# big-nacho/patolette

Measured on AMD Instinct MI355X. Metric: Mpixels/sec quantized (256-color ICtCp + KMeans) at 1 GPU; palette ΔE vs ref, higher is better.
Workload: dtype f64

## Files before the change

include/patolette_amd.h:

```cpp
#ifndef PATOLETTE_AMD_H
#define PATOLETTE_AMD_H

#include <stddef.h>
#include <stdint.h>

#include "patolette.h"

#ifdef __cplusplus
extern "C" {
#endif

int  patolette_amd_device_count(void);
int  patolette_amd_set_device(int ordinal);
const char *patolette_amd_last_error(void);
void *patolette_amd_malloc(size_t bytes);
void patolette_amd_free(void *dptr);
int  patolette_amd_memcpy_h2d(void *dst, const void *src, size_t bytes);
int  patolette_amd_memcpy_d2h(void *dst, const void *src, size_t bytes);
int  patolette_amd_synchronize(void);
void patolette_amd_release_workspace(void);
int  patolette_amd_fill_image(double *d_planar, size_t n, uint64_t seed);
int  patolette_amd_fill_weights(double *d_weights, size_t n, uint64_t seed);

void patolette_amd_device(size_t width, size_t height, const double *d_data, const double *d_weights,
// ... 182 lines not shown
int patolette_amd_set_invariant_sums(int on);
int patolette_amd_set_kmeans_update(int mode);

int patolette_amd_set_split_loop(int mode);
int patolette_amd_set_global_quantiser(int on_device);

int patolette_amd_set_subsample_cache(int on);

int patolette_amd_subsample_indices(size_t n, size_t take, int32_t *out);
int patolette_amd_eigen_sym3(const double a_colmajor[9], double w[3], double z[9]);
int patolette_amd_principal_axis(const double cov6[6], double axis[3]);
int patolette_amd_eigen_sym3_device(const double *a_colmajor, size_t count, double *w, double *z, int *info);
int patolette_amd_debug_gq_table(const double *table, const uint32_t *counts, int weighted, size_t palette_size, int route, int *kbase, int *error,
                                 int *cuts, unsigned char *bucket_table, uint64_t *begin, uint64_t *n, double *sw, double *mean,
                                 uint64_t *prefix_w0, double *prefix, int *cut_table);
int patolette_amd_pow(const double *x, double y, double *out, size_t n);
int patolette_amd_debug_pow(const double *x, double y, double *out, size_t n, int mode);

enum {
    PAMD_SRGB_TO_ICTCP = 0,
    PAMD_SRGB_TO_CIELUV = 1,
    PAMD_ICTCP_TO_REC2020 = 2,
    PAMD_CIELUV_TO_REC2020 = 3,
    PAMD_SRGB_TO_REC2020 = 4,
    PAMD_REC2020_TO_SRGB = 5,
    PAMD_CIELUV_TO_ICTCP = 6
};
int patolette_amd_convert(int which, double *planar, size_t n);
int patolette_amd_debug_convert(int which, const double *planar, const unsigned char *bytes, int channels, double *out, size_t n, int general);

// ... 76 lines not shown
```

patolette_amd/_native.py:

```python
import ctypes as C
import os

HERE = os.path.dirname(os.path.abspath(__file__))
LIB_PATH = os.path.join(HERE, "lib", "libpatolette_amd.so")

dp = C.POINTER(C.c_double)
zp = C.POINTER(C.c_size_t)


class QuantizationOptions(C.Structure):
    _fields_ = [("dither", C.c_bool), ("palette_only", C.c_bool), ("color_space", C.c_int),
                ("kmeans_niter", C.c_int), ("kmeans_max_samples", C.c_size_t), ("verbose", C.c_bool)]


class Stats(C.Structure):
    _fields_ = [(n, C.c_double) for n in ("ms_total", "ms_upload", "ms_convert", "ms_gq", "ms_lq",
                                          "ms_kmeans", "ms_map", "ms_download", "ms_saliency")] + \
               [(n, C.c_size_t) for n in ("n_base_clusters", "n_clusters", "split_evals", "split_px",
                                          "lq_rounds", "kmeans_samples", "dither_segments", "dither_repairs",
                                          "dither_rounds", "dither_through", "dither_jumps", "dither_solo")]

    def as_dict(self):
        return {n: getattr(self, n) for n, _ in self._fields_}

# ... 40 lines not shown
                                        C.c_size_t, C.POINTER(QuantizationOptions), C.POINTER(dp), C.c_void_p, C.c_int,
                                        C.POINTER(C.c_int)]),
    "patolette_amd_slice": (None, [C.c_size_t, C.c_size_t, C.c_size_t, dp, dp, C.c_size_t, C.POINTER(QuantizationOptions),
                                   C.POINTER(Comm), dp, zp, C.POINTER(C.c_int)]),
    "patolette_amd_slice_device": (None, [C.c_size_t, C.c_size_t, C.c_size_t, C.c_void_p, C.c_void_p, C.c_size_t,
                                          C.POINTER(QuantizationOptions), C.POINTER(Comm), dp, C.c_void_p, C.c_int, C.POINTER(C.c_int)]),
    "patolette_amd_set_invariant_sums": (C.c_int, [C.c_int]),
    "patolette_amd_set_kmeans_update": (C.c_int, [C.c_int]),
    "patolette_amd_set_subsample_cache": (C.c_int, [C.c_int]),
    "patolette_amd_subsample_indices": (C.c_int, [C.c_size_t, C.c_size_t, C.POINTER(C.c_int32)]),
    "patolette_amd_eigen_sym3": (C.c_int, [dp, dp, dp]),
    "patolette_amd_principal_axis": (C.c_int, [dp, dp]),
    "patolette_amd_eigen_sym3_device": (C.c_int, [dp, C.c_size_t, dp, dp, C.POINTER(C.c_int)]),
    "patolette_amd_debug_gq_table": (C.c_int, [dp, C.c_void_p, C.c_int, C.c_size_t, C.c_int, C.POINTER(C.c_int), C.POINTER(C.c_int), C.c_void_p,
                                               C.c_void_p, C.c_void_p, C.c_void_p, dp, dp, C.c_void_p, dp, C.c_void_p]),
    "patolette_amd_fill_image": (C.c_int, [C.c_void_p, C.c_size_t, C.c_uint64]),
    "patolette_amd_fill_weights": (C.c_int, [C.c_void_p, C.c_size_t, C.c_uint64]),
    "patolette_amd_device": (None, [C.c_size_t, C.c_size_t, C.c_void_p, C.c_void_p, C.c_size_t,
                                    C.POINTER(QuantizationOptions), dp, C.c_void_p, C.c_int, C.POINTER(C.c_int)]),
    "patolette_amd_quantize": (None, [C.c_size_t, C.c_size_t, dp, dp, C.c_double, C.c_size_t, C.POINTER(QuantizationOptions), dp, zp,
                                      C.POINTER(C.c_int)]),
    "patolette_amd_quantize_rows": (None, [C.c_size_t, C.c_size_t, dp, dp, C.c_double, C.c_size_t, C.POINTER(QuantizationOptions), dp,
                                           zp, C.POINTER(C.c_int)]),
    "patolette_amd_saliency_weights": (C.c_int, [C.c_size_t, C.c_size_t, dp, C.c_double, dp]),
    "patolette_amd_mbd": (C.c_int, [C.c_size_t, C.c_size_t, C.POINTER(C.c_float), C.c_int, C.POINTER(C.c_float)]),
    **_pair("patolette_amd_u8", None, [C.c_size_t, C.c_size_t, C.c_void_p, C.c_int, C.c_void_p, C.c_double, C.c_size_t,
                                       C.POINTER(QuantizationOptions), dp, C.c_void_p, C.c_void_p, C.c_int, C.c_void_p, C.POINTER(C.c_int)]),
    **_pair("patolette_amd_frames_u8", None, [C.c_size_t, C.c_size_t, C.c_size_t, C.c_void_p, C.c_int, C.c_void_p, C.c_double, C.c_size_t,
                                              C.POINTER(QuantizationOptions), dp, C.c_void_p, C.c_void_p, C.c_int, C.c_void_p,
                                              C.POINTER(C.c_int)]),
# ... 141 lines not shown
    ctab = np.zeros((13, 513), dtype=np.int32) if details else None
    vp = lambda a: a.ctypes.data_as(C.c_void_p) if a is not None else None
    rc = lib().patolette_amd_debug_gq_table(t.ctypes.data_as(dp), vp(c), 1 if weighted else 0, int(palette_size), int(route), C.byref(kbase),
                                            C.byref(error), vp(cuts), vp(lut), vp(begin), vp(n), sw.ctypes.data_as(dp), mean.ctypes.data_as(dp),
                                            vp(pw0), pre.ctypes.data_as(dp) if details else None, vp(ctab))
    if rc != 0:
        raise RuntimeError("patolette_amd_debug_gq_table: %d (%s)" % (rc, last_error()))
    k = kbase.value
    out = dict(kbase=k, error=error.value, cuts=[int(v) for v in cuts[:k + 1]] if k else [], bucket_table=lut, begin=begin[:k].copy(),
               n=n[:k].copy(), sw=sw[:k].copy(), mean=mean[:k].copy())
    if details:
        out.update(prefix_w0=pw0, prefix=pre, cut_table=ctab)
    return out


def last_cluster_centers():
    import numpy as np
    n = lib().patolette_amd_last_cluster_centers(None, 0)
    out = np.zeros((max(1, n), 3), order="F")
    lib().patolette_amd_last_cluster_centers(out.ctypes.data_as(dp), max(1, n))
    return np.ascontiguousarray(out[:n])


def profile(enable=True, only=None, sample=1):
    lib().patolette_amd_profile_only(only.encode() if only else None)
    lib().patolette_amd_profile_sample(int(sample) if only else 1)
    lib().patolette_amd_profile_enable(1 if enable else 0)


def profile_results():
# ... 11 lines not shown
```

patolette_amd/csrc/map.h:

```cpp
#pragma once

#include "common.h"

namespace pamd {

struct NNWork {
    DevBuf<unsigned char> lut;
    DevBuf<unsigned long long> keys;
    DevBuf<unsigned char> clist;
    DevBuf<unsigned int> mid;
    DevBuf<double> dtab;
    DevBuf<unsigned int> dside;
    PinBuf<unsigned int> hrep;
    DevBuf<double> dsort;
    DevBuf<unsigned int> dpos;
    size_t order_w = 0, order_h = 0; int order_dev = -1;
    DevBuf<unsigned int> dmpos;
    DevBuf<unsigned int> dmcnt;
    DevBuf<unsigned char> dsmap;
    DevBuf<unsigned char> dflag;
    size_t dither_segments = 0, dither_repairs = 0, dither_rounds = 0;
    size_t dither_through = 0;
    size_t dither_jumps = 0;
    size_t dither_solo = 0;
// ... 2 lines not shown
    int side_dev = -1;
    struct LaneTables { bool valid = false; double lo[3][3], hi[3][3], inv[3][3]; int G[3]; float amb, amb_p, amb_x; } lane_tables;
    NNWork() = default;
    NNWork(const NNWork &) = delete;
    NNWork &operator=(const NNWork &) = delete;
    ~NNWork() {
        if (ev_fork) (void)hipEventDestroy(ev_fork);
        if (ev_join) (void)hipEventDestroy(ev_join);
        if (ev_join2) (void)hipEventDestroy(ev_join2);
        if (side_stream) (void)hipStreamDestroy(side_stream);
        if (side_stream2) (void)hipStreamDestroy(side_stream2);
    }
};
void launch_nn_map(const double *d_colors, size_t plane_stride, size_t n, const double *d_pal, int k,
                   void *d_out, int elem_bytes, const double *lo, const double *hi, NNWork &w, hipStream_t s);
int nn_debug_route(int route);
bool nn_map_u8_applies(size_t n, int k);
void launch_nn_map_u8(const unsigned char *d_px, int channels, size_t n, const double *d_pal, int k, void *d_out, int elem_bytes, NNWork &w, hipStream_t s);

struct DitherJob {
    const double *planes = nullptr;
    size_t plane_stride = 0;
    int which = -1;
    const unsigned char *bytes = nullptr;
    int channels = 3;
    size_t frames = 1, width = 0, height = 0;
    const int *cpos = nullptr;
    size_t opaque = 0;
    const unsigned *mpos = nullptr;
    const double *d_pal = nullptr, *h_pal = nullptr;
// ... 20 lines not shown
```

patolette_amd/csrc/map.hip:

```cpp
#include "map.h"
#include "compact.h"
#include "dither_host.h"
#include "dither_slots.h"

#include <algorithm>
#include <atomic>
#include <cmath>
#include <mutex>
#include <type_traits>

#define PAMD_POW_TABLES_IN_LDS
#include "color_device.h"
#include "devutil.h"

namespace pamd {

template <typename OutT>
__global__ __launch_bounds__(256) void k_nn_map(const double *__restrict__ c, size_t N, size_t n, const double *__restrict__ pal, int k,
                                                OutT *__restrict__ out) {
    const double *palx = pal, *paly = pal + k, *palz = pal + 2 * k;
    const size_t stride = (size_t)gridDim.x * blockDim.x;
    for (size_t i = (size_t)blockIdx.x * blockDim.x + threadIdx.x; i < n; i += stride) {
        const double x = c[i], y = c[N + i], z = c[2 * N + i];
        double bd = INFINITY; int best = 0;
// ... 788 lines not shown
    const int blocks = (int)std::min<size_t>((size_t)num_cus(), ceil_div(n, (size_t)64 * WAVES * P));
    KTIME("k_nn_map_u8", s, ((double)channels + sizeof(OutT)) * n);
    hipLaunchKernelGGL((k_nn_map_mid<OutT, P, WAVES, NNSrcU8>), blocks, 64 * WAVES, lds, s, NNSrcU8{d_px, (size_t)channels}, n, d_pal, k, g, (const unsigned int *)w.mid.p,
                       (const float4 *)(w.mid.p + ncell / 8), (const unsigned char *)l1, (const unsigned char *)l2, out);
}
void launch_nn_map_u8(const unsigned char *d_px, int channels, size_t n, const double *d_pal, int k, void *d_out, int elem_bytes, NNWork &w, hipStream_t s) {
    if (!nn_map_u8_applies(n, k)) throw HipError("patolette_amd: the byte-source map kernel takes 2^22 .. 2^32 pixels and 8 .. 256 palette rows");
    if (channels != 3 && channels != 4) throw HipError("patolette_amd: 8-bit pixels have 3 or 4 channels");
    w.lane_tables.valid = false;
    if (elem_bytes == 1) launch_nn_mid_u8<unsigned char>(d_px, channels, n, d_pal, k, (unsigned char *)d_out, w, s);
    else if (elem_bytes == 4) launch_nn_mid_u8<unsigned int>(d_px, channels, n, d_pal, k, (unsigned int *)d_out, w, s);
    else throw HipError("patolette_amd: the byte-source map kernel writes 1- or 4-byte elements");
    HIP_CHECK(hipGetLastError());
}

void launch_nn_map(const double *d_colors, size_t plane_stride, size_t n, const double *d_pal, int k, void *d_out, int elem_bytes,
                   const double *lo, const double *hi, NNWork &w, hipStream_t s) {
    if (elem_bytes != 1 && elem_bytes != 4 && elem_bytes != 8) throw HipError("patolette_amd: map element size must be 1, 4 or 8");
    w.lane_tables.valid = false;
    const int cls = nn_size_class(n);
    bool use_lut = cls >= 1 && k >= 8 && k <= 4096;
    double blo[3] = {0, 0, 0}, bhi[3] = {0, 0, 0};
    if (use_lut) {
        if (lo && hi) { for (int a = 0; a < 3; a++) { blo[a] = lo[a]; bhi[a] = hi[a]; } }
        else {
            w.keys.reserve(6);
            unsigned long long init[6] = {~0ULL, ~0ULL, ~0ULL, 0ULL, 0ULL, 0ULL}, got[6];
            HIP_CHECK(hipMemcpyAsync(w.keys.p, init, sizeof init, hipMemcpyHostToDevice, s));
            { KTIME("k_minmax3", s, 24.0 * n); hipLaunchKernelGGL(k_minmax3, stream_blocks(n, 16), 256, 0, s, d_colors, plane_stride, n, w.keys.p); }
            HIP_CHECK(hipMemcpyAsync(got, w.keys.p, sizeof got, hipMemcpyDeviceToHost, s));
// ... 1649 lines not shown
```

patolette_amd/csrc/pipeline.hip:

```cpp
#include <algorithm>
#include <functional>
#include <chrono>
#include <cmath>
#include <atomic>
#include <memory>
#include <mutex>
#include <thread>
#include <future>
#include <type_traits>

#include "color_device.h"
#include "common.h"
#include "host_math.h"
#include "kmeans.h"
#include "map.h"
#include "ordered.h"
#include "delta.h"
#include "measure.h"
#include "lzw.h"
#include "lzw_near.h"
#include "deflate.h"
#include "hist.h"
#include "saliency.h"
#include "quant.h"
// ... 817 lines not shown
    size_t total = 0, begin = 0;
    patolette_amd__Comm comm{};
};

struct Engine {
    int device = -1;
    hipStream_t stream = nullptr;
    const Shard *shard = nullptr;
    bool invariant = false;
    DevBuf<unsigned char> commbuf;
    PinBuf<unsigned char> h_comm;
    DevBuf<int> shard_ids;
    PinBuf<float> h_cent;
    PinBuf<ConvertStats> h_cstats;
    hipEvent_t ev_stats = nullptr;
    hipStream_t stream2 = nullptr;
    hipEvent_t ev_up[2] = {nullptr, nullptr}, ev_join = nullptr;
    size_t prep_N = 0, prep_planes = 0;
    DevBuf<double> src, wsrc, cvt, bufA, bufB, aux;
    DevBuf<unsigned short> bkt;
    DevBuf<NodeDev> nodes;
    DevBuf<NodeIn> stage_in;
    DevBuf<NodeOut> stage_out;
    DevBuf<int> ids, round_nodes, node_tile0;
    DevBuf<Tile> tilesA, tilesP;
    DevBuf<double> hist, sum6, dpal;
    DevBuf<unsigned long long> hsize, tileoff;
    DevBuf<unsigned int> hcount, tilecnt;
    DevBuf<unsigned char> lut, dmap, src8, pal8, quant8;
    DevBuf<unsigned char> dl_maps, dl_shown;
// ... 39 lines not shown
    PinBuf<double> h_pal;
    DevBuf<LqCtl> lqctl;
    PinBuf<LqHead> h_lqhead;
    PinBuf<LqRec> h_lqrec;
    PinBuf<LqCen> h_lqcen;
    std::vector<LqRec> lq_rec_local;
    std::vector<LqCommit> lq_commits;
    bool trace_pending = false;
    size_t lq_hint_N = 0, lq_hint_K = 0; int lq_hint_rounds = 0;
    DevBuf<int> perm_dev;
    size_t perm_N = 0, perm_nx = 0;
    PinBuf<int32_t> h_perm;
    size_t hperm_N = 0, hperm_nx = 0;
    hm::PermScratch perm_ws;
    std::future<void> perm_job;
    patolette_amd__Stats stats{};
    double ms_saliency = 0.0;
    std::string last_error;
    std::vector<double> map_palette;
    patolette_amd__SplitTrace trace_hdr{};
    std::vector<patolette_amd__SplitRecord> trace;
    std::vector<double> cluster_centers;

    void init() {
        if (stream) return;
        int cnt = 0;
        if (hipGetDeviceCount(&cnt) != hipSuccess || cnt <= 0)
            throw HipError("patolette_amd: no HIP device available (this library has no CPU fallback)");
        if (device < 0) { HIP_CHECK(hipGetDevice(&device)); }
        HIP_CHECK(hipSetDevice(device));
        HIP_CHECK(hipStreamCreateWithFlags(&stream, hipStreamNonBlocking));
    }
    void sync() { HIP_CHECK(hipStreamSynchronize(stream)); if (ktimer().enabled) ktimer().collect(); }
    ~Engine() {
        if (stream) { (void)hipSetDevice(device); (void)hipStreamSynchronize(stream); if (ev_stats) (void)hipEventDestroy(ev_stats);
                      for (hipEvent_t e : {ev_up[0], ev_up[1], ev_join}) if (e) (void)hipEventDestroy(e);
                      if (stream2) (void)hipStreamDestroy(stream2);
                      (void)hipStreamDestroy(stream); }
    }
};

namespace {
std::mutex g_pool_mu;
std::vector<Engine *> g_pool;
thread_local int tl_invariant = -1;
bool invariant_default() {
    static const bool env = getenv("PAMD_INVARIANT_SUMS") && atoi(getenv("PAMD_INVARIANT_SUMS")) != 0;
    return tl_invariant < 0 ? env : tl_invariant != 0;
}
Engine *pool_acquire(int device, bool invariant) {
// ... 143 lines not shown

static void get_nodes(Engine &E, const std::vector<int> &ids, std::vector<NodeOut> &recs) {
    const int n = (int)ids.size();
    recs.resize(n);
    if (!n) return;
    E.stage_out.reserve(n); E.ids.reserve(n); E.h_stage_out.reserve(n); E.h_ids_get.reserve(n);
    std::memcpy(E.h_ids_get.p, ids.data(), n * sizeof(int));
    HIP_CHECK(hipMemcpyAsync(E.ids.p, E.h_ids_get.p, n * sizeof(int), hipMemcpyHostToDevice, E.stream));
    hipLaunchKernelGGL(k_get_nodes, (n + 63) / 64, 64, 0, E.stream, E.nodes.p, E.stage_out.p, E.ids.p, n);
    HIP_CHECK(hipGetLastError());
    HIP_CHECK(hipMemcpyAsync(E.h_stage_out.p, E.stage_out.p, n * sizeof(NodeOut), hipMemcpyDeviceToHost, E.stream));
    E.sync();
    std::memcpy(recs.data(), E.h_stage_out.p, n * sizeof(NodeOut));
}

static void get_nodes_dev(Engine &E, const int *d_ids, int n, std::vector<NodeOut> &recs) {
    recs.resize(n);
    if (!n) return;
    E.h_stage_out.reserve(n);
    hipLaunchKernelGGL(k_get_nodes, (n + 63) / 64, 64, 0, E.stream, E.nodes.p, E.h_stage_out.p, d_ids, n);
    HIP_CHECK(hipGetLastError());
    E.sync();
    std::memcpy(recs.data(), E.h_stage_out.p, n * sizeof(NodeOut));
}

static void absorb_moments(HNode &h, const NodeOut &d) {
    for (int q = 0; q < 6; q++) h.cov6[q] = d.acc[q][0] + d.acc[q][1];
    h.dist = d.acc[6][0] + d.acc[6][1];
}

static bool node_axis(const HNode &h, double axis[3]) {
    if (h.axis_state != 0) {
        for (int j = 0; j < 3; j++) axis[j] = h.axis[j];
        return h.axis_state > 0;
    }
    double c6[6];
    for (int q = 0; q < 6; q++) c6[q] = h.cov6[q] / h.sw;
// ... 120 lines not shown
        }
        launch_hist(qlq, false, E.tilesA.p, ntA_ub, 0, E.nodes.p, E.hist.p, E.hsize.p, E.hcount.p, s, !rev, false, dyn, px_src);
        launch_cut(weighted, E.nodes.p, d_round, kLqRoundCap, E.hist.p, E.hsize.p, E.hcount.p, E.lut.p, s, dyn, nr_src);
        launch_partition(qlq, E.tilesP.p, ntP_ub, 0, d_round, d_tP0, kLqRoundCap, E.nodes.p, E.lut.p, E.tilecnt.p, E.tileoff.p, true, s, inv_sums, rev, dyn, px_src);
        enq++;
        control();
    };
    control();
    int want = (E.lq_hint_N == N && E.lq_hint_K == K && E.lq_hint_rounds > 0) ? E.lq_hint_rounds : 9;
    const bool fault_full = g_debug_fault.load(std::memory_order_relaxed) == 4;
    if (fault_full) want = 3;
    for (;;) {
        while (enq < want) round();
        hipLaunchKernelGGL(k_lq_export, 16, 256, 0, s, (const LqCtl *)c, head, E.h_lqrec.p, E.h_lqcen.p);
        HIP_CHECK(hipGetLastError());
        E.sync();
        if (fault_full) return -2;
        if (head->done) break;
        want = enq + 2;
    }
    if (head->error == 2) return -2;
    if (head->error == 3) return -1;
    if (kbase < 0) kbase = E.h_gqout.p->kbase;
    E.lq_hint_N = N; E.lq_hint_K = K; E.lq_hint_rounds = head->rounds;
    LqReplay rp;
    const double t_rp0 = now_ms();
    E.lq_rec_local.resize((size_t)head->nnodes);
    std::memcpy(E.lq_rec_local.data(), E.h_lqrec.p, (size_t)head->nnodes * sizeof(LqRec));
    const int fault = g_debug_fault.load(std::memory_order_relaxed);
    const bool replay_ok = lq_replay(E.lq_rec_local.data(), kbase, first_base, K, kDelta, fault, rp);
    const double t_rp1 = now_ms();
// ... 605 lines not shown
    return v < 0 ? env : v != 0;
}
static bool km_domain_ok(const double bound_x, const double bound_c, const bool weighted, const double bound_w, const double min_w, const size_t nx) {
    const double fmax = 3.4028234663852886e38, fmin = 1.1754943508222875e-38;
    const double B = std::max(1.0, std::max(bound_x, bound_c)), m = (double)std::min<size_t>(nx, (size_t)1 << 25);
    if (!(B < fmax) || !(bound_w < fmax)) return false;
    double Cb = 8.0 * B;
    if (weighted) {
        if (min_w > 0 && min_w < fmin) return false;
        const double by_n = std::exp(std::min((double)nx * 0x1p-23, 700.0)) * B;
        Cb = 4.0 * (min_w > 0 ? std::min(by_n, 4.0 * m * (std::max(bound_w, min_w) / min_w) * B) : by_n);
    }
    Cb += 8.0;
    return 16.0 * Cb * Cb <= fmax && 4.0 * m * std::max(bound_w, 1.0) * B <= fmax;
}
static void kmeans_refine(Engine &E, size_t N, bool weighted, std::vector<double> &centers, size_t k, int niter, size_t max_samples,
                          bool nonfinite, unsigned long long largest_cluster, double bound_x, double bound_w, double min_w = 0, bool bad_w = false) {
    hipStream_t s = E.stream;
    E.km.route = 0;
    const KmSums sums_v{bound_x, bound_w};
    const KmSums *sums = km_update_order_free() ? &sums_v : nullptr;
    std::vector<float> cent(3 * k);
    for (size_t i = 0; i < k; i++) for (int j = 0; j < 3; j++) cent[3 * i + j] = (float)centers[(size_t)j * k + i];
    const size_t min_samples = 256 * 256;
    const size_t ms = std::max(max_samples, min_samples);
    const int mppc = (int)(ms / k);
    const Shard *sh = E.shard;
    const size_t Nt = sh ? sh->total : N;
    auto expect_longest = [&](size_t nx_) { return (size_t)((double)largest_cluster / (double)(Nt ? Nt : 1) * (double)nx_); };
    bool ok = Nt >= k && !nonfinite && !bad_w;
    size_t nx = Nt;
    E.stats.kmeans_samples = 0;
    const bool sub = ok && Nt > k * (size_t)mppc;
    if (sub) nx = k * (size_t)mppc;
// ... 19 lines not shown
                HIP_CHECK(hipMemcpy(f.data() + 2 * k, E.km.sz.p, k * sizeof(float), hipMemcpyDeviceToHost));
                for (size_t i = 0; i < k; i++) for (int j = 0; j < 3; j++) cent[3 * i + j] = f[(size_t)j * k + i];
            } else {
                HIP_CHECK(hipMemcpyAsync(E.km.cent.p, cent.data(), 3 * k * sizeof(float), hipMemcpyHostToDevice, s));
                HIP_CHECK(hipStreamSynchronize(s));
                kmeans_iterate(E.km, nx, (int)k, weighted, niter, s, expect_longest(nx), sums);
                HIP_CHECK(hipMemcpyAsync(cent.data(), E.km.cent.p, 3 * k * sizeof(float), hipMemcpyDeviceToHost, s));
                E.sync();
                E.stats.kmeans_samples = nx;
            }
        } else if (nx == k) {
            std::vector<double> first(3 * k);
            for (int j = 0; j < 3; j++) HIP_CHECK(hipMemcpy(first.data() + (size_t)j * k, E.cvt.p + (size_t)j * N, k * sizeof(double), hipMemcpyDeviceToHost));
            for (size_t i = 0; i < k; i++) for (int j = 0; j < 3; j++) cent[3 * i + j] = (float)first[(size_t)j * k + i];
        } else {
            kmeans_gather(E.cvt.p, N, weighted, dperm, nx, E.km, s);
            E.h_cent.reserve(3 * k);
            std::memcpy(E.h_cent.p, cent.data(), 3 * k * sizeof(float));
            HIP_CHECK(hipMemcpyAsync(E.km.cent.p, E.h_cent.p, 3 * k * sizeof(float), hipMemcpyHostToDevice, s));
            kmeans_iterate(E.km, nx, (int)k, weighted, niter, s, expect_longest(nx), sums);
            HIP_CHECK(hipMemcpyAsync(E.h_cent.p, E.km.cent.p, 3 * k * sizeof(float), hipMemcpyDeviceToHost, s));
            E.sync();
            std::memcpy(cent.data(), E.h_cent.p, 3 * k * sizeof(float));
            E.stats.kmeans_samples = nx;
        }
    }
    for (size_t i = 0; i < k; i++) for (int j = 0; j < 3; j++) centers[(size_t)j * k + i] = (double)cent[3 * i + j];
}

static void palette_rows(std::vector<double> &pal, size_t len, void (*f)(double[3])) {
    for (size_t i = 0; i < len; i++) {
        double c[3] = {pal[i], pal[len + i], pal[2 * len + i]};
        f(c);
        pal[i] = c[0]; pal[len + i] = c[1]; pal[2 * len + i] = c[2];
    }
}
// ... 91 lines not shown
}

static void write_palette(double *out, size_t K, size_t off, const std::vector<double> &pal, size_t rows) {
    for (size_t j = 0; j < K * 3; j++) out[j] = j % K < off ? 0.0 : -1.0;
    for (int j = 0; j < 3; j++) for (size_t i = 0; i < rows; i++) out[K * (size_t)j + off + i] = pal[(size_t)j * rows + i];
}

static void add_dither_stats(Engine &E) {
    E.stats.dither_segments += E.nn.dither_segments; E.stats.dither_repairs += E.nn.dither_repairs; E.stats.dither_rounds += E.nn.dither_rounds;
    E.stats.dither_through += E.nn.dither_through; E.stats.dither_jumps += E.nn.dither_jumps; E.stats.dither_solo += E.nn.dither_solo;
}
static bool map_touched(bool dither, size_t width, size_t height) { return !(dither && std::max(width, height) <= 1); }

static void run_device(Engine &E, size_t width, size_t height, Pixels px, const double *d_weights, size_t K,
                       const patolette__QuantizationOptions *opt, double *palette, void *d_map, int map_elem, const DitherMask *mask = nullptr,
                       const Frames *frames = nullptr) {
    hipStream_t s = E.stream;
    const size_t N = width * height;
    const bool weighted = d_weights != nullptr;
    const double t_start = now_ms();
    WsGuard wg(&E.stream, &E.stream2);
    E.stats = patolette_amd__Stats{};
    E.prep_N = 0;
    ws_prepare(E, N, K, weighted, opt->verbose);
    if (opt->kmeans_niter > 0) subsample_start(E, E.shard ? E.shard->total : N, K, opt->kmeans_max_samples);
    double t0 = now_ms();
    if (E.shard && opt->dither && !opt->palette_only)
        throw HipError("patolette_amd: dithering walks the whole image along one curve; it is not available per slice");
    const ConvertPlan cp = convert_plan(E, opt, N);
    if (!px.converted) convert_pixels(E, cp, px, N, s);
    if (weighted) {
        HIP_CHECK(hipMemcpyAsync(E.cvt.p + 3 * N, d_weights, N * sizeof(double), hipMemcpyDeviceToDevice, s));
        launch_weight_stats(d_weights, N, E.cstats.p, s);
    }
    Bounds bnd = read_bounds(E, weighted, [&] { gq_prepare(E, N, weighted); });
    bnd.have_sum = cp.sumk.M0 != 0.0;
    bnd.have_mom = cp.momk.M0 != 0.0;
    E.stats.ms_convert = now_ms() - t0;

    if (opt->verbose) printf("patolette ======== Palette generation \n");
    std::vector<double> pal;
    size_t len = 0;
    unsigned long long largest_cluster = 0;
    if (quantize_clusters(E, N, K, weighted, bnd, pal, len, opt->verbose, &largest_cluster) != 0) throw HipError("internal quantization error");

    t0 = now_ms();
    if (opt->kmeans_niter > 0) {
        if (opt->verbose) printf("patolette ======== KMeans refinement\n");
        kmeans_refine(E, N, weighted, pal, len, opt->kmeans_niter, opt->kmeans_max_samples, bnd.nonfinite, largest_cluster, bnd.cmax, bnd.wmax, bnd.wmin, bnd.bad_w);
    }
    E.stats.ms_kmeans = now_ms() - t0;

    t0 = now_ms();
    if (!opt->palette_only) {
        E.dpal.reserve(3 * len);
        if (opt->verbose) printf(opt->dither ? "patolette ======== Dithering\n" : "patolette ======== NN mapping\n");
        if (opt->dither) {
            int pix = PAMD_SRGB_TO_REC2020;
            void (*pf)(double[3]) = hm::color::srgb_to_rec2020;
            if (opt->color_space == patolette__CIELuv) { pix = PAMD_CIELUV_TO_REC2020; pf = hm::color::cieluv_to_rec2020; }
            else if (opt->color_space == patolette__ICtCp) { pix = PAMD_ICTCP_TO_REC2020; pf = hm::color::ictcp_to_rec2020; }
            palette_rows(pal, len, pf);
            E.map_palette = pal;
            if (d_map) {
// ... 208 lines not shown
    E.stats.ms_upload = in.ms_upload;
    E.stats.ms_download = now_ms() - t_out;
    E.stats.ms_total += E.ms_saliency + in.ms_upload + E.stats.ms_download;
}

static void run_host(Engine &E, size_t width, size_t height, const double *data, const double *weights, double tile_size,
                     size_t K, const patolette__QuantizationOptions *opt, double *palette, size_t *palette_map, bool rows = false,
                     void *d_map_out = nullptr) {
    const size_t N = width * height;
    const double t_start = now_ms();
    WsGuard wg(&E.stream, &E.stream2);
    const int me = map_elem_for(K);
    if (!opt->palette_only && !d_map_out) E.dmap.reserve(N * (size_t)me);
    const QuantInput in = quant_input(E, t_start, Pixels{data, nullptr, 3, rows}, false, true, 1, width, height, weights, tile_size, K, opt);
    std::vector<double> pal(3 * K);
    run_device(E, width, height, in.px, in.d_w, K, opt, pal.data(), d_map_out ? d_map_out : (void *)E.dmap.p, me);
    const double t_out = now_ms();
    if (!opt->palette_only && !d_map_out && map_touched(opt->dither, width, height)) download_map_widened(E, E.dmap.p, me, N, palette_map);
    std::memcpy(palette, pal.data(), 3 * K * sizeof(double));
    quant_stats(E, in, t_out);
}

static void download_map(const void *d_map, int me, size_t N, void *map_out, int map_elem_out) {
    if (map_elem_out == me) { HIP_CHECK(hipMemcpy(map_out, d_map, N * (size_t)me, hipMemcpyDeviceToHost)); return; }
    std::vector<unsigned char> tmp(N * (size_t)me);
    HIP_CHECK(hipMemcpy(tmp.data(), d_map, tmp.size(), hipMemcpyDeviceToHost));
    given_elems_out(tmp.data(), me, map_out, map_elem_out, 0, N);
}

static HipError named_error(const char *name, const char *text) { return HipError(std::string(name) + ": " + text); }
static const char *const kBadDeviceMapElem = "patolette_amd: device map_elem_bytes must be 1 for K <= 256, else 4";
// ... 853 lines not shown
                                        : "patolette_amd_slice: unusable arguments (empty slice, slice outside the image, missing buffer)");
        body(E);
    });
    if (Ep) Ep->shard = nullptr;
}

static void host_entry(bool rows, size_t width, size_t height, const double *data, const double *weights, double tile_size, size_t palette_size,
                       const patolette__QuantizationOptions *options, double *palette, size_t *palette_map, int *exit_code) {
    *exit_code = validate(width, height, palette_size);
    if (*exit_code != 0) return;
    *exit_code = guarded([&](Engine &E) { run_host(E, width, height, data, weights, tile_size, palette_size, options, palette, palette_map, rows); });
}
static void device_entry_run(Engine &E, size_t width, size_t height, const double *d_data, const double *d_weights, size_t palette_size,
                             const patolette__QuantizationOptions *options, double *palette, void *d_map, int map_elem_bytes) {
    std::vector<double> pal(3 * palette_size);
    run_device(E, width, height, Pixels{d_data, nullptr, 3}, d_weights, palette_size, options, pal.data(), d_map, map_elem_bytes);
    std::memcpy(palette, pal.data(), 3 * palette_size * sizeof(double));
}

extern "C" {

void patolette(size_t width, size_t height, const double *data, const double *weights, size_t palette_size,
               const patolette__QuantizationOptions *options, double *palette, size_t *palette_map, int *exit_code) {
    host_entry(false, width, height, data, weights, 0.0, palette_size, options, palette, palette_map, exit_code);
}

void patolette_amd_quantize(size_t width, size_t height, const double *data, const double *weights, double tile_size,
                            size_t palette_size, const patolette__QuantizationOptions *options, double *palette,
                            size_t *palette_map, int *exit_code) {
    host_entry(false, width, height, data, weights, tile_size, palette_size, options, palette, palette_map, exit_code);
}
// ... 865 lines not shown
        E.sync();
        if (prefix_w0) std::memcpy(prefix_w0, h_pre->w0, sizeof(h_pre->w0));
        if (prefix) std::memcpy(prefix, h_pre->t, sizeof(h_pre->t));
        if (cut_table) std::memcpy(cut_table, h_g->cut, sizeof(h_g->cut));
        if (o.error) { *error = 1; std::memset(bucket_table, 0, kBuckets); return 0; }
        *kbase = o.kbase;
        for (int j = 0; j <= o.kbase && j < 14; j++) cuts[j] = o.cuts[j];
        for (int j = 0; j < o.kbase; j++) {
            const NodeDev &c = h_nodes[1 + j];
            begin[j] = c.begin; n[j] = c.n; sw[j] = c.sw;
            for (int q = 0; q < 3; q++) mean[3 * j + q] = c.mean[q];
        }
        return 0;
    });
}
int patolette_amd_eigen_sym3(const double a_colmajor[9], double w[3], double z[9]) {
    std::memcpy(z, a_colmajor, 9 * sizeof(double));
    return hm::eigen_sym3(z, w);
}

void patolette_amd_batch(size_t count, size_t width, size_t height, const double *const *data, const double *const *weights,
                         double tile_size, size_t palette_size, const patolette__QuantizationOptions *options, double *const *palettes,
                         size_t *const *palette_maps, int *exit_codes) {
    batch_impl(false, count, width, height, data, weights, tile_size, palette_size, options, palettes, palette_maps, exit_codes);
}
void patolette_amd_batch_rows(size_t count, size_t width, size_t height, const double *const *rows, const double *const *weights,
                              double tile_size, size_t palette_size, const patolette__QuantizationOptions *options,
                              double *const *palettes, size_t *const *palette_maps, int *exit_codes) {
    batch_impl(true, count, width, height, rows, weights, tile_size, palette_size, options, palettes, palette_maps, exit_codes);
}
// ... 206 lines not shown
```

Baseline: 3234.

## Overlap KMeans gather with host syncs and hand centroids to NN map on device

Defers the KMeans sample gather into a callback that runs while the host waits on earlier local-quantizer syncs, so the gather overlaps with waiting instead of running serially later. When the palette goes to a device map, KMeans centroids are converted to a double palette by a new kernel and NN mapping is launched right away, skipping a host round-trip. Map work buffers are pre-reserved. A debug entry point for LQ selection is also added. This adds complex state (lambda, precomputed-gather validity) and timing-split logic that could go stale across calls.

Result: no change. 3255 (median of 6 runs) (+0.7%).

```diff
diff --git a/include/patolette_amd.h b/include/patolette_amd.h
--- a/include/patolette_amd.h
+++ b/include/patolette_amd.h
@@ -220,6 +220,10 @@
 int patolette_amd_debug_gq_table(const double *table, const uint32_t *counts, int weighted, size_t palette_size, int route, int *kbase, int *error,
                                  int *cuts, unsigned char *bucket_table, uint64_t *begin, uint64_t *n, double *sw, double *mean,
                                  uint64_t *prefix_w0, double *prefix, int *cut_table);
+int patolette_amd_debug_lq_select(const int *params, double *rec_val, int *rec_left, int *rec_kn, double *np, const int *nparent, int *leaves,
+                                  int *round_ids, const int *cids, const uint64_t *node_n, const uint64_t *node_gn, const double *node_dist,
+                                  int *node_child0, const int *node_axis_state, int *node_slot, int *node_nchild, double *node_bink,
+                                  int *cids_next, int *tA0, int *tP0, int *head, uint64_t *head_u64, double *head_f64);
 int patolette_amd_pow(const double *x, double y, double *out, size_t n);
 int patolette_amd_debug_pow(const double *x, double y, double *out, size_t n, int mode);
 
diff --git a/patolette_amd/_native.py b/patolette_amd/_native.py
--- a/patolette_amd/_native.py
+++ b/patolette_amd/_native.py
@@ -78,6 +78,7 @@
     "patolette_amd_eigen_sym3_device": (C.c_int, [dp, C.c_size_t, dp, dp, C.POINTER(C.c_int)]),
     "patolette_amd_debug_gq_table": (C.c_int, [dp, C.c_void_p, C.c_int, C.c_size_t, C.c_int, C.POINTER(C.c_int), C.POINTER(C.c_int), C.c_void_p,
                                                C.c_void_p, C.c_void_p, C.c_void_p, dp, dp, C.c_void_p, dp, C.c_void_p]),
+    "patolette_amd_debug_lq_select": (C.c_int, [C.c_void_p] * 23),
     "patolette_amd_fill_image": (C.c_int, [C.c_void_p, C.c_size_t, C.c_uint64]),
     "patolette_amd_fill_weights": (C.c_int, [C.c_void_p, C.c_size_t, C.c_uint64]),
     "patolette_amd_device": (None, [C.c_size_t, C.c_size_t, C.c_void_p, C.c_void_p, C.c_size_t,
@@ -249,6 +250,47 @@
     return out
 
 
+LQ_NODE_CAP, LQ_ROUND_CAP = 4352, 512
+
+
+def debug_lq_select(state):
+    import numpy as np
+    nn, nl, nc, nrp = (int(state[k]) for k in ("nnodes", "nleaves", "ncids", "nr_prev"))
+    params = np.array([nn, nl, nc, nrp] + [int(state[k]) for k in ("M", "rounds", "neval", "call", "e_lin", "e_quad")], dtype=np.int32)
+
+    def arr(name, dtype, n, room=None):
+        a = np.ascontiguousarray(state[name], dtype=dtype).reshape(-1)
+        if a.size != n:
+            raise ValueError("debug_lq_select: %s must hold %d entries" % (name, n))
+        out = np.full(max(room or n, 1), 0 if dtype is np.uint64 else -1, dtype=dtype)
+        out[:n] = a
+        return out
+    o = dict(rec_val=arr("rec_val", np.float64, nn), rec_left=arr("rec_left", np.int32, nn), rec_kn=arr("rec_kn", np.int32, nn),
+             np=arr("np", np.float64, nn), nparent=arr("nparent", np.int32, nn), leaves=arr("leaves", np.int32, nl),
+             round_ids=arr("round_ids", np.int32, nrp, LQ_ROUND_CAP), cids=arr("cids", np.int32, nc),
+             node_n=arr("node_n", np.uint64, nn), node_gn=arr("node_gn", np.uint64, nn), node_dist=arr("node_dist", np.float64, nn),
+             node_child0=arr("node_child0", np.int32, nn), node_axis_state=arr("node_axis_state", np.int32, nn),
+             node_slot=np.zeros(max(nn, 1), dtype=np.int32), node_nchild=np.zeros(max(nn, 1), dtype=np.int32),
+             node_bink=np.zeros((max(nn, 1), 4)), cids_next=np.zeros(2 * LQ_ROUND_CAP, dtype=np.int32),
+             tA0=np.zeros(LQ_ROUND_CAP + 1, dtype=np.int32), tP0=np.zeros(LQ_ROUND_CAP + 1, dtype=np.int32))
+    head, hu, hf = np.zeros(11, dtype=np.int32), np.zeros(2, dtype=np.uint64), np.zeros(3)
+    order = ("rec_val", "rec_left", "rec_kn", "np", "nparent", "leaves", "round_ids", "cids", "node_n", "node_gn", "node_dist", "node_child0",
+             "node_axis_state", "node_slot", "node_nchild", "node_bink", "cids_next", "tA0", "tP0")
+    vp = lambda a: a.ctypes.data_as(C.c_void_p)
+    rc = lib().patolette_amd_debug_lq_select(vp(params), *[vp(o[k]) for k in order], vp(head), vp(hu), vp(hf))
+    if rc != 0:
+        raise RuntimeError("patolette_amd_debug_lq_select: %d (%s)" % (rc, last_error()))
+    for k in ("nparent", "cids", "node_n", "node_gn", "node_dist", "node_axis_state"):
+        del o[k]
+    for k in ("rec_val", "rec_left", "rec_kn", "np", "node_child0", "node_slot", "node_nchild", "node_bink"):
+        o[k] = o[k][:nn]
+    o["leaves"] = o["leaves"][:nl]
+    names = ("done", "error", "rounds", "nnodes", "neval", "nleaves", "ncids_next", "dyn_nr", "dyn_ntA", "dyn_ntP", "dyn_pad")
+    o.update({k: int(v) for k, v in zip(names, head)})
+    o.update(split_evals=int(hu[0]), split_px=int(hu[1]), tau=float(hf[0]), round_px=float(hf[1]), round_nr=float(hf[2]))
+    return o
+
+
 def last_cluster_centers():
     import numpy as np
     n = lib().patolette_amd_last_cluster_centers(None, 0)
diff --git a/patolette_amd/csrc/map.h b/patolette_amd/csrc/map.h
--- a/patolette_amd/csrc/map.h
+++ b/patolette_amd/csrc/map.h
@@ -40,6 +40,7 @@
 };
 void launch_nn_map(const double *d_colors, size_t plane_stride, size_t n, const double *d_pal, int k,
                    void *d_out, int elem_bytes, const double *lo, const double *hi, NNWork &w, hipStream_t s);
+void nn_map_reserve(size_t n, int k, NNWork &w);
 int nn_debug_route(int route);
 bool nn_map_u8_applies(size_t n, int k);
 void launch_nn_map_u8(const unsigned char *d_px, int channels, size_t n, const double *d_pal, int k, void *d_out, int elem_bytes, NNWork &w, hipStream_t s);
diff --git a/patolette_amd/csrc/map.hip b/patolette_amd/csrc/map.hip
--- a/patolette_amd/csrc/map.hip
+++ b/patolette_amd/csrc/map.hip
@@ -826,6 +826,15 @@
     HIP_CHECK(hipGetLastError());
 }
 
+void nn_map_reserve(size_t n, int k, NNWork &w) {
+    const int cls = nn_size_class(n);
+    if (!(cls >= 1 && k >= 8)) return;
+    const int G = cls == 2 ? 64 : 32, ncell = G * G * G;
+    w.lut.reserve((size_t)ncell * (k <= 256 ? 32 : 64));
+    if (G == 64) w.mid.reserve((size_t)(ncell / 8) + 257 * 4);
+    w.clist.reserve((size_t)(ncell / 64) * (1 + kCoarseMax) * 2);
+}
+
 void launch_nn_map(const double *d_colors, size_t plane_stride, size_t n, const double *d_pal, int k, void *d_out, int elem_bytes,
                    const double *lo, const double *hi, NNWork &w, hipStream_t s) {
     if (elem_bytes != 1 && elem_bytes != 4 && elem_bytes != 8) throw HipError("patolette_amd: map element size must be 1, 4 or 8");
diff --git a/patolette_amd/csrc/pipeline.hip b/patolette_amd/csrc/pipeline.hip
--- a/patolette_amd/csrc/pipeline.hip
+++ b/patolette_amd/csrc/pipeline.hip
@@ -855,6 +855,7 @@
     PinBuf<float> h_cent;
     PinBuf<ConvertStats> h_cstats;
     hipEvent_t ev_stats = nullptr;
+    hipEvent_t ev_stage[2] = {nullptr, nullptr};
     hipStream_t stream2 = nullptr;
     hipEvent_t ev_up[2] = {nullptr, nullptr}, ev_join = nullptr;
     size_t prep_N = 0, prep_planes = 0;
@@ -924,6 +925,8 @@
     size_t hperm_N = 0, hperm_nx = 0;
     hm::PermScratch perm_ws;
     std::future<void> perm_job;
+    std::function<void()> km_early;
+    struct KmPre { bool valid = false; size_t N = 0, nx = 0; bool weighted = false, sub = false; } km_pre;
     patolette_amd__Stats stats{};
     double ms_saliency = 0.0;
     std::string last_error;
@@ -944,6 +947,7 @@
     void sync() { HIP_CHECK(hipStreamSynchronize(stream)); if (ktimer().enabled) ktimer().collect(); }
     ~Engine() {
         if (stream) { (void)hipSetDevice(device); (void)hipStreamSynchronize(stream); if (ev_stats) (void)hipEventDestroy(ev_stats);
+                      for (hipEvent_t e : ev_stage) if (e) (void)hipEventDestroy(e);
                       for (hipEvent_t e : {ev_up[0], ev_up[1], ev_join}) if (e) (void)hipEventDestroy(e);
                       if (stream2) (void)hipStreamDestroy(stream2);
                       (void)hipStreamDestroy(stream); }
@@ -1117,13 +1121,27 @@
     std::memcpy(recs.data(), E.h_stage_out.p, n * sizeof(NodeOut));
 }
 
+static void km_early_run(Engine &E) {
+    if (!E.km_early) return;
+    const std::function<void()> f = std::move(E.km_early);
+    E.km_early = nullptr;
+    f();
+}
+static void sync_then_km_early(Engine &E) {
+    if (!E.km_early || ktimer().enabled) { km_early_run(E); E.sync(); return; }
+    if (!E.ev_stats) HIP_CHECK(hipEventCreateWithFlags(&E.ev_stats, hipEventDisableTiming));
+    HIP_CHECK(hipEventRecord(E.ev_stats, E.stream));
+    km_early_run(E);
+    HIP_CHECK(hipEventSynchronize(E.ev_stats));
+}
+
 static void get_nodes_dev(Engine &E, const int *d_ids, int n, std::vector<NodeOut> &recs) {
     recs.resize(n);
     if (!n) return;
     E.h_stage_out.reserve(n);
     hipLaunchKernelGGL(k_get_nodes, (n + 63) / 64, 64, 0, E.stream, E.nodes.p, E.h_stage_out.p, d_ids, n);
     HIP_CHECK(hipGetLastError());
-    E.sync();
+    sync_then_km_early(E);
     std::memcpy(recs.data(), E.h_stage_out.p, n * sizeof(NodeOut));
 }
 
@@ -1274,7 +1292,7 @@
         while (enq < want) round();
         hipLaunchKernelGGL(k_lq_export, 16, 256, 0, s, (const LqCtl *)c, head, E.h_lqrec.p, E.h_lqcen.p);
         HIP_CHECK(hipGetLastError());
-        E.sync();
+        sync_then_km_early(E);
         if (fault_full) return -2;
         if (head->done) break;
         want = enq + 2;
@@ -1910,10 +1928,20 @@
     Cb += 8.0;
     return 16.0 * Cb * Cb <= fmax && 4.0 * m * std::max(bound_w, 1.0) * B <= fmax;
 }
+__global__ void k_km_cent_to_pal(const float *__restrict__ cent, const int k, double *__restrict__ pal) {
+    const int t = blockIdx.x * blockDim.x + threadIdx.x;
+    if (t < 3 * k) pal[(size_t)(t % 3) * k + t / 3] = (double)cent[t];
+}
+static void kmeans_take_centroids(Engine &E, std::vector<double> &centers, size_t k) {
+    for (size_t i = 0; i < k; i++) for (int j = 0; j < 3; j++) centers[(size_t)j * k + i] = (double)E.h_cent.p[3 * i + j];
+}
 static void kmeans_refine(Engine &E, size_t N, bool weighted, std::vector<double> &centers, size_t k, int niter, size_t max_samples,
-                          bool nonfinite, unsigned long long largest_cluster, double bound_x, double bound_w, double min_w = 0, bool bad_w = false) {
+                          bool nonfinite, unsigned long long largest_cluster, double bound_x, double bound_w, double min_w = 0, bool bad_w = false,
+                          double *d_pal_out = nullptr, bool *pending = nullptr) {
     hipStream_t s = E.stream;
     E.km.route = 0;
+    const Engine::KmPre pre = E.km_pre;
+    E.km_pre.valid = false;
     const KmSums sums_v{bound_x, bound_w};
     const KmSums *sums = km_update_order_free() ? &sums_v : nullptr;
     std::vector<float> cent(3 * k);
@@ -1963,12 +1991,17 @@
             for (int j = 0; j < 3; j++) HIP_CHECK(hipMemcpy(first.data() + (size_t)j * k, E.cvt.p + (size_t)j * N, k * sizeof(double), hipMemcpyDeviceToHost));
             for (size_t i = 0; i < k; i++) for (int j = 0; j < 3; j++) cent[3 * i + j] = (float)first[(size_t)j * k + i];
         } else {
-            kmeans_gather(E.cvt.p, N, weighted, dperm, nx, E.km, s);
+            if (!(pre.valid && pre.N == N && pre.nx == nx && pre.weighted == weighted && pre.sub == sub)) kmeans_gather(E.cvt.p, N, weighted, dperm, nx, E.km, s);
             E.h_cent.reserve(3 * k);
             std::memcpy(E.h_cent.p, cent.data(), 3 * k * sizeof(float));
             HIP_CHECK(hipMemcpyAsync(E.km.cent.p, E.h_cent.p, 3 * k * sizeof(float), hipMemcpyHostToDevice, s));
             kmeans_iterate(E.km, nx, (int)k, weighted, niter, s, expect_longest(nx), sums);
+            if (d_pal_out && pending) {
+                hipLaunchKernelGGL(k_km_cent_to_pal, (unsigned)((3 * k + 255) / 256), 256, 0, s, (const float *)E.km.cent.p, (int)k, d_pal_out);
+                HIP_CHECK(hipGetLastError());
+            }
             HIP_CHECK(hipMemcpyAsync(E.h_cent.p, E.km.cent.p, 3 * k * sizeof(float), hipMemcpyDeviceToHost, s));
+            if (d_pal_out && pending) { E.stats.kmeans_samples = nx; *pending = true; return; }
             E.sync();
             std::memcpy(cent.data(), E.h_cent.p, 3 * k * sizeof(float));
             E.stats.kmeans_samples = nx;
@@ -2090,7 +2123,7 @@
 
 static void run_device(Engine &E, size_t width, size_t height, Pixels px, const double *d_weights, size_t K,
                        const patolette__QuantizationOptions *opt, double *palette, void *d_map, int map_elem, const DitherMask *mask = nullptr,
-                       const Frames *frames = nullptr) {
+                       const Frames *frames = nullptr, bool device_handoff = false) {
     hipStream_t s = E.stream;
     const size_t N = width * height;
     const bool weighted = d_weights != nullptr;
@@ -2100,6 +2133,30 @@
     E.prep_N = 0;
     ws_prepare(E, N, K, weighted, opt->verbose);
     if (opt->kmeans_niter > 0) subsample_start(E, E.shard ? E.shard->total : N, K, opt->kmeans_max_samples);
+    struct KmEarlyGuard { Engine &E; ~KmEarlyGuard() { E.km_early = nullptr; E.km_pre.valid = false; } } km_early_guard{E};
+    E.km_early = nullptr; E.km_pre.valid = false;
+    if (opt->kmeans_niter > 0 && !E.shard && K > 0 && N >= K) {
+        const size_t ms = std::max(opt->kmeans_max_samples, (size_t)(256 * 256));
+        const size_t nxK = K * (size_t)(int)(ms / K);
+        const bool sub = N > nxK;
+        const size_t nx = sub ? nxK : N;
+        if (!(sub && nx < K + 1) && nx != K) {
+            E.km.reserve(std::min(N, ms), (int)K);
+            if (sub && !(E.perm_N == N && E.perm_nx >= nx)) {
+                E.perm_N = 0; E.perm_nx = 0;
+                E.perm_dev.reserve(std::max(std::min(N, ms), E.hperm_N == N ? E.hperm_nx : (size_t)0));
+            }
+            Engine *pe = &E;
+            E.km_early = [pe, N, nx, sub, weighted] {
+                const int *dperm = sub ? subsample_list(*pe, N, nx, pe->stream) : nullptr;
+                kmeans_gather(pe->cvt.p, N, weighted, dperm, nx, pe->km, pe->stream);
+                pe->km_pre = Engine::KmPre{true, N, nx, weighted, sub};
+            };
+        }
+    }
+    const bool handoff = device_handoff && opt->kmeans_niter > 0 && !opt->palette_only && !opt->dither && d_map && !E.shard && !mask && !frames &&
+                         opt->color_space != patolette__CIELuv;
+    if (handoff) nn_map_reserve(N, (int)std::min<size_t>(K, (size_t)1 << 30), E.nn);
     double t0 = now_ms();
     if (E.shard && opt->dither && !opt->palette_only)
         throw HipError("patolette_amd: dithering walks the whole image along one curve; it is not available per slice");
@@ -2121,9 +2178,32 @@
     if (quantize_clusters(E, N, K, weighted, bnd, pal, len, opt->verbose, &largest_cluster) != 0) throw HipError("internal quantization error");
 
     t0 = now_ms();
+    bool km_pending = false;
     if (opt->kmeans_niter > 0) {
         if (opt->verbose) printf("patolette ======== KMeans refinement\n");
-        kmeans_refine(E, N, weighted, pal, len, opt->kmeans_niter, opt->kmeans_max_samples, bnd.nonfinite, largest_cluster, bnd.cmax, bnd.wmax, bnd.wmin, bnd.bad_w);
+        kmeans_refine(E, N, weighted, pal, len, opt->kmeans_niter, opt->kmeans_max_samples, bnd.nonfinite, largest_cluster, bnd.cmax, bnd.wmax, bnd.wmin, bnd.bad_w,
+                      handoff ? E.dpal.p : nullptr, handoff ? &km_pending : nullptr);
+    }
+    if (km_pending) {
+        for (hipEvent_t &e : E.ev_stage) if (!e) HIP_CHECK(hipEventCreate(&e));
+        HIP_CHECK(hipEventRecord(E.ev_stage[0], s));
+        if (opt->verbose) printf("patolette ======== NN mapping\n");
+        launch_nn_map(E.cvt.p, N, N, E.dpal.p, (int)len, d_map, map_elem, bnd.lo, bnd.hi, E.nn, s);
+        HIP_CHECK(hipEventRecord(E.ev_stage[1], s));
+        HIP_CHECK(hipEventSynchronize(E.ev_stage[0]));
+        kmeans_take_centroids(E, pal, len);
+        E.map_palette = pal;
+        palette_rows(pal, len, hm::color::ictcp_to_rec2020);
+        palette_rows(pal, len, hm::color::rec2020_to_srgb);
+        E.sync();
+        float ms_map = 0.f;
+        HIP_CHECK(hipEventElapsedTime(&ms_map, E.ev_stage[0], E.ev_stage[1]));
+        const double both = now_ms() - t0;
+        E.stats.ms_map = std::min((double)ms_map, both);
+        E.stats.ms_kmeans = both - E.stats.ms_map;
+        write_palette(palette, K, 0, pal, len);
+        E.stats.ms_total = now_ms() - t_start;
+        return;
     }
     E.stats.ms_kmeans = now_ms() - t0;
 
@@ -2362,7 +2442,7 @@
     if (!opt->palette_only && !d_map_out) E.dmap.reserve(N * (size_t)me);
     const QuantInput in = quant_input(E, t_start, Pixels{data, nullptr, 3, rows}, false, true, 1, width, height, weights, tile_size, K, opt);
     std::vector<double> pal(3 * K);
-    run_device(E, width, height, in.px, in.d_w, K, opt, pal.data(), d_map_out ? d_map_out : (void *)E.dmap.p, me);
+    run_device(E, width, height, in.px, in.d_w, K, opt, pal.data(), d_map_out ? d_map_out : (void *)E.dmap.p, me, nullptr, nullptr, true);
     const double t_out = now_ms();
     if (!opt->palette_only && !d_map_out && map_touched(opt->dither, width, height)) download_map_widened(E, E.dmap.p, me, N, palette_map);
     std::memcpy(palette, pal.data(), 3 * K * sizeof(double));
@@ -3246,7 +3326,7 @@
 static void device_entry_run(Engine &E, size_t width, size_t height, const double *d_data, const double *d_weights, size_t palette_size,
                              const patolette__QuantizationOptions *options, double *palette, void *d_map, int map_elem_bytes) {
     std::vector<double> pal(3 * palette_size);
-    run_device(E, width, height, Pixels{d_data, nullptr, 3}, d_weights, palette_size, options, pal.data(), d_map, map_elem_bytes);
+    run_device(E, width, height, Pixels{d_data, nullptr, 3}, d_weights, palette_size, options, pal.data(), d_map, map_elem_bytes, nullptr, nullptr, true);
     std::memcpy(palette, pal.data(), 3 * palette_size * sizeof(double));
 }
 
@@ -4142,6 +4222,77 @@
         return 0;
     });
 }
+int patolette_amd_debug_lq_select(const int *params, double *rec_val, int *rec_left, int *rec_kn, double *np, const int *nparent, int *leaves,
+                                  int *round_ids, const int *cids, const uint64_t *node_n, const uint64_t *node_gn, const double *node_dist,
+                                  int *node_child0, const int *node_axis_state, int *node_slot, int *node_nchild, double *node_bink,
+                                  int *cids_next, int *tA0, int *tP0, int *head, uint64_t *head_u64, double *head_f64) {
+    if (!params || !rec_val || !rec_left || !rec_kn || !np || !nparent || !leaves || !round_ids || !node_n || !node_gn || !node_dist ||
+        !node_child0 || !node_axis_state || !node_slot || !node_nchild || !node_bink || !cids_next || !tA0 || !tP0 || !head || !head_u64 || !head_f64)
+        return -1;
+    const int nn = params[0], nleaves = params[1], ncids = params[2], nr_prev = params[3], M = params[4], rounds = params[5], neval = params[6],
+              call = params[7], e_lin = params[8], e_quad = params[9];
+    if (nn < 0 || nn > kLqNodeCap || nleaves < 0 || nleaves > kLqNodeCap || ncids < 0 || ncids > nleaves || ncids > 2 * kLqRoundCap || nr_prev < 0 ||
+        nr_prev > kLqRoundCap || rounds < 0 || call < 0 || (ncids && !cids))
+        return -1;
+    for (int i = 0; i < nn; i++) if (nparent[i] < -1 || nparent[i] >= nn) return -1;
+    for (int i = 0; i < nleaves; i++) if (leaves[i] < 0 || leaves[i] >= nn) return -1;
+    for (int i = 0; i < ncids; i++) if (cids[i] < 0 || cids[i] >= nn) return -1;
+    for (int i = 0; i < nr_prev; i++) {
+        const int id = round_ids[i];
+        if (id < 0 || id >= nn) return -1;
+        if (node_axis_state[id] >= 0 && (node_child0[id] < 0 || node_child0[id] + 1 >= nn)) return -1;
+    }
+    return guarded([&](Engine &E) -> int {
+        hipStream_t s = E.stream;
+        const int cur = call & 1, nxt = cur ^ 1;
+        const size_t nnb = (size_t)std::max(nn, 1);
+        std::vector<NodeDev> h_nodes(nnb);
+        std::memset(static_cast<void *>(h_nodes.data()), 0, nnb * sizeof(NodeDev));
+        for (int i = 0; i < nn; i++) {
+            NodeDev &d = h_nodes[i];
+            d.n = node_n[i]; d.gn = node_gn[i]; d.dist = node_dist[i]; d.child0 = node_child0[i]; d.axis_state = node_axis_state[i];
+            d.slot = -1; d.nchild = -1;
+        }
+        auto h_c = std::make_unique<LqCtl>();
+        LqCtl &c = *h_c;
+        std::memset(static_cast<void *>(&c), 0xFF, sizeof(LqCtl));
+        c.h.done = 0; c.h.error = 0; c.h.rounds = rounds; c.h.nnodes = nn; c.h.neval = neval; c.h.pad = 0; c.h.split_evals = 0ULL; c.h.split_px = 0ULL;
+        c.h.tau = -1.0;
+        for (int r = 0; r < kLqMaxRounds; r++) { c.h.round_px[r] = -1.0; c.h.round_nr[r] = -1.0; }
+        c.K = M; c.M = M; c.nleaves = nleaves - ncids; c.pad = 0; c.ncids[cur] = ncids; c.ncids[nxt] = -1;
+        c.dyn = RoundDyn{nr_prev, 0, 0, 0};
+        for (int i = 0; i < nleaves; i++) c.leaves[i] = leaves[i];
+        for (int i = 0; i < nr_prev; i++) c.round_ids[i] = round_ids[i];
+        for (int i = 0; i < ncids; i++) c.cids[cur][i] = cids[i];
+        for (int i = 0; i < nn; i++) { c.nparent[i] = nparent[i]; c.np[i] = np[i]; c.nrec[i] = LqRec{rec_val[i], rec_left[i], rec_kn[i]}; }
+        DevBuf<NodeDev> d_nodes; DevBuf<LqCtl> d_c;
+        d_nodes.reserve(nnb); d_c.reserve(1);
+        HIP_CHECK(hipMemcpyAsync(d_nodes.p, h_nodes.data(), nnb * sizeof(NodeDev), hipMemcpyHostToDevice, s));
+        HIP_CHECK(hipMemcpyAsync(d_c.p, &c, sizeof(LqCtl), hipMemcpyHostToDevice, s));
+        hipLaunchKernelGGL(k_lq_select, 1, 256, 0, s, d_nodes.p, d_c.p, call, e_lin, e_quad);
+        HIP_CHECK(hipGetLastError());
+        HIP_CHECK(hipMemcpyAsync(h_nodes.data(), d_nodes.p, nnb * sizeof(NodeDev), hipMemcpyDeviceToHost, s));
+        HIP_CHECK(hipMemcpyAsync(&c, d_c.p, sizeof(LqCtl), hipMemcpyDeviceToHost, s));
+        E.sync();
+        for (int i = 0; i < nn; i++) {
+            const NodeDev &d = h_nodes[i];
+            node_child0[i] = d.child0; node_slot[i] = d.slot; node_nchild[i] = d.nchild;
+            node_bink[4 * i] = d.klin.M0; node_bink[4 * i + 1] = d.klin.M1; node_bink[4 * i + 2] = d.kquad.M0; node_bink[4 * i + 3] = d.kquad.M1;
+            rec_val[i] = c.nrec[i].val; rec_left[i] = c.nrec[i].left; rec_kn[i] = c.nrec[i].kn; np[i] = c.np[i];
+        }
+        for (int i = 0; i < nleaves; i++) leaves[i] = c.leaves[i];
+        for (int i = 0; i < kLqRoundCap; i++) round_ids[i] = c.round_ids[i];
+        for (int i = 0; i < 2 * kLqRoundCap; i++) cids_next[i] = c.cids[nxt][i];
+        for (int i = 0; i <= kLqRoundCap; i++) { tA0[i] = c.tA0[i]; tP0[i] = c.tP0[i]; }
+        const int hv[11] = {c.h.done, c.h.error, c.h.rounds, c.h.nnodes, c.h.neval, c.nleaves, c.ncids[nxt], c.dyn.nr, c.dyn.ntA, c.dyn.ntP, c.dyn.pad};
+        for (int i = 0; i < 11; i++) head[i] = hv[i];
+        head_u64[0] = c.h.split_evals; head_u64[1] = c.h.split_px;
+        head_f64[0] = c.h.tau;
+        head_f64[1] = rounds < kLqMaxRounds ? c.h.round_px[rounds] : -1.0;
+        head_f64[2] = rounds < kLqMaxRounds ? c.h.round_nr[rounds] : -1.0;
+        return 0;
+    });
+}
 int patolette_amd_eigen_sym3(const double a_colmajor[9], double w[3], double z[9]) {
     std::memcpy(z, a_colmajor, 9 * sizeof(double));
     return hm::eigen_sym3(z, w);
```
